# advimman/lama

Measured on NVIDIA H100. Metric: images/sec FFCResNetGenerator @512x512 bs32, higher is better.
Workload: dtype bf16x3(f32 accumulate)

## Files before the change

### include/ffc_b200.h

```cpp
#ifndef FFC_B200_H_
#define FFC_B200_H_

#include <stddef.h>
#include <stdint.h>

#ifdef __cplusplus
extern "C" {
#endif

#define FFCB_VERSION 117

enum {
  FFCB_OK = 0,
  FFCB_EINVAL = -1,
  FFCB_EARCH = -2,
  FFCB_ECUDA = -3,
  FFCB_ENOMEM = -4
};

enum { FFCB_F32 = 0, FFCB_BF16X2 = 1 };
enum { FFCB_ACT_NONE = 0, FFCB_ACT_RELU = 1, FFCB_ACT_SIGMOID = 2, FFCB_ACT_TANH = 3 };
enum { FFCB_BORDER_ZERO = 0, FFCB_BORDER_REFLECT = 1 };
enum {
  FFCB_MATH_FP32 = 0,
  FFCB_MATH_BF16X3 = 1
};

typedef void* ffcb_stream_t;

typedef struct {
  void* ptr;
  int64_t sb, sy, sx;
  int64_t lo_off;
  int32_t B, H, W, C;
  int32_t fmt;
  int32_t pad;
  int32_t reflect_border;
  int32_t window;
  int32_t cg;
  int32_t tile;
  int64_t sg;
} ffcb_tensor;

typedef struct {
  int32_t src, dy, dx, c0, nch;
} ffcb_kseg;

#define FFCB_MAX_KSEG 64

typedef struct {
  ffcb_tensor in[2];
  ffcb_tensor out;
  ffcb_tensor addend;
  const void* weight;
  const float* shift;
  int32_t n_out;
  int32_t stride;
  int32_t border;
  int32_t act;
  int32_t nseg;
  int32_t math;
  int32_t addend_post;
  int32_t _reserved;
  ffcb_kseg seg[FFCB_MAX_KSEG];
} ffcb_conv_desc;

int ffcb_version(void);
const char* ffcb_last_error(void);
int ffcb_check_device(int device);
void ffcb_shutdown(void);

int ffcb_conv(const ffcb_conv_desc* desc, ffcb_stream_t stream);

enum { FFCB_PLAN_FLAT = 0, FFCB_PLAN_SPATIAL = 1, FFCB_PLAN_ROWS = 2, FFCB_PLAN_HALO = 3 };
typedef struct {
  int32_t kind;
  int32_t il, po, ring;
  int32_t bn, tw, th, stages;
  int64_t m_tiles;
  int32_t n_tiles;
  int32_t _reserved;
} ffcb_conv_plan_info;
int ffcb_conv_plan(const ffcb_conv_desc* desc, ffcb_conv_plan_info* info);

int ffcb_stem_conv7(const float* x_nchw, int B, int Cin, int H, int W, const float* w, const float* shift,
                    int N, const ffcb_tensor* out, ffcb_stream_t stream);

int ffcb_stem_pack(const float* x_nchw, int B, int Cin, int H, int W, const ffcb_tensor* packed, ffcb_stream_t stream);

int ffcb_head_conv7(const ffcb_tensor* in, const float* w, const float* bias, int N, int act, float* y_nchw,
                    ffcb_stream_t stream);

size_t ffcb_fft2_workspace_bytes(int B, int H, int W, int C);
int ffcb_rfft2(const ffcb_tensor* in, const ffcb_tensor* spec, void* ws, size_t ws_bytes, ffcb_stream_t stream);
int ffcb_irfft2(const ffcb_tensor* spec, const ffcb_tensor* residual , const ffcb_tensor* out,
                void* ws, size_t ws_bytes, ffcb_stream_t stream);

int ffcb_head_gather7(const ffcb_tensor* q, const float* bias, int N, int act, float* y_nchw, ffcb_stream_t stream);

int ffcb_stem_pack_u8(const uint8_t* image_hwc, const uint8_t* mask_hw, int B, int H0, int W0,
                      const ffcb_tensor* packed, ffcb_stream_t stream);
int ffcb_head_gather7_blend_u8(const ffcb_tensor* q, const float* bias, int act, const uint8_t* image_hwc,
                               const uint8_t* mask_hw, int H0, int W0, uint8_t* out_hwc, ffcb_stream_t stream);

int ffcb_nchw_to_nhwc(const float* x_nchw, int B, int C, int H, int W, const ffcb_tensor* out, ffcb_stream_t stream);
int ffcb_nhwc_to_nchw(const ffcb_tensor* in, float* y_nchw, ffcb_stream_t stream);
int ffcb_fill_reflect_border(const ffcb_tensor* t, ffcb_stream_t stream);
// ... 34 lines not shown
```

### lama_b200/_lib.py

```python
import ctypes as C
import os

HERE = os.path.dirname(os.path.abspath(__file__))
LIB_PATH = os.path.join(HERE, "libffc_b200.so")

OK, EINVAL, EARCH, ECUDA, ENOMEM = 0, -1, -2, -3, -4
F32, BF16X2 = 0, 1
ACT_NONE, ACT_RELU, ACT_SIGMOID, ACT_TANH = 0, 1, 2, 3
BORDER_ZERO, BORDER_REFLECT = 0, 1
MATH_FP32, MATH_BF16X3 = 0, 1
MAX_KSEG = 64
PLAN_FLAT, PLAN_SPATIAL, PLAN_ROWS, PLAN_HALO = 0, 1, 2, 3
VERSION = 117


class Tensor(C.Structure):
    _fields_ = [("ptr", C.c_void_p), ("sb", C.c_int64), ("sy", C.c_int64), ("sx", C.c_int64),
                ("lo_off", C.c_int64), ("B", C.c_int32), ("H", C.c_int32), ("W", C.c_int32), ("C", C.c_int32),
                ("fmt", C.c_int32), ("pad", C.c_int32), ("reflect_border", C.c_int32), ("window", C.c_int32),
                ("cg", C.c_int32), ("tile", C.c_int32), ("sg", C.c_int64)]


class KSeg(C.Structure):
    _fields_ = [("src", C.c_int32), ("dy", C.c_int32), ("dx", C.c_int32), ("c0", C.c_int32), ("nch", C.c_int32)]


class ConvDesc(C.Structure):
    _fields_ = [("inp", Tensor * 2), ("out", Tensor), ("addend", Tensor), ("weight", C.c_void_p),
                ("shift", C.c_void_p), ("n_out", C.c_int32), ("stride", C.c_int32), ("border", C.c_int32),
                ("act", C.c_int32), ("nseg", C.c_int32), ("math", C.c_int32), ("addend_post", C.c_int32),
                ("_reserved", C.c_int32), ("seg", KSeg * MAX_KSEG)]


class ConvPlanInfo(C.Structure):
    _fields_ = [("kind", C.c_int32), ("il", C.c_int32), ("po", C.c_int32), ("ring", C.c_int32), ("bn", C.c_int32),
                ("tw", C.c_int32), ("th", C.c_int32), ("stages", C.c_int32), ("m_tiles", C.c_int64),
                ("n_tiles", C.c_int32), ("_reserved", C.c_int32)]


_PT = C.POINTER(Tensor)
SIGNATURES = {
    "ffcb_version": (C.c_int, []),
    "ffcb_last_error": (C.c_char_p, []),
    "ffcb_check_device": (C.c_int, [C.c_int]),
    "ffcb_shutdown": (None, []),
    "ffcb_conv": (C.c_int, [C.POINTER(ConvDesc), C.c_void_p]),
# ... 69 lines not shown
```

### lama_b200/csrc/conv_tc.cu

```cuda
#include <cuda.h>
#include <stdlib.h>

#include <type_traits>

#include "common.cuh"

namespace ffcb {
namespace {

constexpr int BM = 128;
constexpr int BK = 64;
constexpr int WG_K = 16;
constexpr int kThreads = 384;
constexpr int kConsumers = 256;
constexpr int kTileABytes = BM * BK * 2;
constexpr int kMaxStages = 8;
constexpr int kBarBytes = 1024;
constexpr int kSmemLimit = 227 * 1024;

struct TcParams {
  View out, addend;
  const float* shift;
  int N, act, addend_post;
  int BN, num_n_tiles;
// ... 140 lines not shown
__device__ __forceinline__ void wgmma_n128(float* d, uint64_t da, uint64_t db, uint32_t scale_d) {
  asm volatile(
      "{\n\t.reg .pred p;\n\tsetp.ne.b32 p, %66, 0;\n\t"
      "wgmma.mma_async.sync.aligned.m64n128k16.f32.bf16.bf16 {"
      "%0, %1, %2, %3, %4, %5, %6, %7, %8, %9, %10, %11, %12, %13, %14, %15, "
      "%16, %17, %18, %19, %20, %21, %22, %23, %24, %25, %26, %27, %28, %29, %30, %31, "
      "%32, %33, %34, %35, %36, %37, %38, %39, %40, %41, %42, %43, %44, %45, %46, %47, "
      "%48, %49, %50, %51, %52, %53, %54, %55, %56, %57, %58, %59, %60, %61, %62, %63"
      "}, %64, %65, p, 1, 1, 0, 0;\n\t}\n"
      : "+f"(d[0]), "+f"(d[1]), "+f"(d[2]), "+f"(d[3]), "+f"(d[4]), "+f"(d[5]), "+f"(d[6]), "+f"(d[7]),
        "+f"(d[8]), "+f"(d[9]), "+f"(d[10]), "+f"(d[11]), "+f"(d[12]), "+f"(d[13]), "+f"(d[14]), "+f"(d[15]),
        "+f"(d[16]), "+f"(d[17]), "+f"(d[18]), "+f"(d[19]), "+f"(d[20]), "+f"(d[21]), "+f"(d[22]), "+f"(d[23]),
        "+f"(d[24]), "+f"(d[25]), "+f"(d[26]), "+f"(d[27]), "+f"(d[28]), "+f"(d[29]), "+f"(d[30]), "+f"(d[31]),
        "+f"(d[32]), "+f"(d[33]), "+f"(d[34]), "+f"(d[35]), "+f"(d[36]), "+f"(d[37]), "+f"(d[38]), "+f"(d[39]),
        "+f"(d[40]), "+f"(d[41]), "+f"(d[42]), "+f"(d[43]), "+f"(d[44]), "+f"(d[45]), "+f"(d[46]), "+f"(d[47]),
        "+f"(d[48]), "+f"(d[49]), "+f"(d[50]), "+f"(d[51]), "+f"(d[52]), "+f"(d[53]), "+f"(d[54]), "+f"(d[55]),
        "+f"(d[56]), "+f"(d[57]), "+f"(d[58]), "+f"(d[59]), "+f"(d[60]), "+f"(d[61]), "+f"(d[62]), "+f"(d[63])
      : "l"(da), "l"(db), "r"(scale_d));
}
template <int BN>
__device__ __forceinline__ void wgmma_bn(float* d, uint64_t da, uint64_t db, uint32_t scale_d) {
  static_assert(BN == 32 || BN == 64 || BN == 96 || BN == 128, "N tile");
  if constexpr (BN == 32) wgmma_n32(d, da, db, scale_d);
  else if constexpr (BN == 64) wgmma_n64(d, da, db, scale_d);
  else if constexpr (BN == 96) wgmma_n96(d, da, db, scale_d);
  else wgmma_n128(d, da, db, scale_d);
}

struct TileCoord {
  int b, y0, x0;
  long long m0;
};

__device__ __forceinline__ TileCoord tile_coord(const TcParams& p, long long m_tile) {
  TileCoord t;
  if (p.flat) {
    t.m0 = m_tile * BM;
    t.b = 0; t.y0 = 0; t.x0 = 0;
  } else {
    const int per_img = p.tiles_x * p.tiles_y;
    t.b = (int)(m_tile / per_img);
    const int r = (int)(m_tile - (long long)t.b * per_img);
    t.y0 = (r / p.tiles_x) * p.TH;
    t.x0 = (r % p.tiles_x) * p.TW;
    t.m0 = 0;
  }
  return t;
}

template <bool IL, bool PO, bool RR, bool HALO, int BN>
__global__ void __launch_bounds__(kThreads, 1)
conv_tc_kernel(const __grid_constant__ TcParams p, const __grid_constant__ CUtensorMap map_in0,
               const __grid_constant__ CUtensorMap map_in1, const __grid_constant__ CUtensorMap map_w) {
  extern __shared__ __align__(1024) uint8_t smem_raw[];
  uint8_t* smem = reinterpret_cast<uint8_t*>((reinterpret_cast<uintptr_t>(smem_raw) + 1023) & ~(uintptr_t)1023);
  const int w_bytes = p.BN * BK * 2;
  const int stage_bytes = RR ? 2 * p.rr_a_bytes : HALO ? 2 * w_bytes : 2 * kTileABytes + 2 * w_bytes;
  uint8_t* w_res = smem;
  uint8_t* a_buf = smem;
  if constexpr (RR) smem += p.rr_w_bytes;
  if constexpr (HALO) smem += (size_t)4 * p.halo_a_bytes;
  uint64_t* bars = reinterpret_cast<uint64_t*>(smem + (size_t)p.stages * stage_bytes);
  uint64_t* full = bars;
  uint64_t* empty = bars + kMaxStages;
  uint64_t* w_bar = bars + 2 * kMaxStages;
  uint64_t* a_full = bars + 2 * kMaxStages + 1;
  uint64_t* a_empty = a_full + 2;

  const int warp = threadIdx.x >> 5, lane = threadIdx.x & 31;

  if (warp == 0 && lane == 0) {
    prefetch_tmap(&map_in0);
    prefetch_tmap(&map_in1);
    prefetch_tmap(&map_w);
  }
  if (warp == 1 && lane == 0) {
    for (int s = 0; s < p.stages; ++s) { mbar_init(&full[s], 1); mbar_init(&empty[s], kConsumers); }
    if constexpr (RR) mbar_init(w_bar, 1);
    if constexpr (HALO)
      for (int s = 0; s < 2; ++s) { mbar_init(&a_full[s], 1); mbar_init(&a_empty[s], kConsumers); }
// ... 96 lines not shown
              uint8_t* st = smem + (size_t)stage * stage_bytes;
              mbar_expect_tx(&full[stage], (uint32_t)stage_bytes);
              const int cc = g.c0 + j * BK;
              if (IL && il) {
                const long long blk = p.flat ? (tc.m0 >> 7)
                                             : (long long)tc.b * p.a_tiles_per_image[g.src] + ((tc.y0 * p.out.W) >> 7);
                const unsigned short* src = p.a_ptr[g.src] + blk * p.a_sg[g.src] + (long long)(cc >> 3) * 1024;
                bulk_load(st, src, kTileABytes, &full[stage]);
                bulk_load(st + kTileABytes, src + p.a_lo[g.src], kTileABytes, &full[stage]);
              } else if (p.flat) {
                tma_load_3d(st, map, &full[stage], cc, (int)tc.m0, 0);
                tma_load_3d(st + kTileABytes, map, &full[stage], cc, (int)tc.m0, 1);
              } else {
                tma_load_5d(st, map, &full[stage], cc, cx, cy, tc.b, 0);
                tma_load_5d(st + kTileABytes, map, &full[stage], cc, cx, cy, tc.b, 1);
              }
              tma_load_3d(st + 2 * kTileABytes, &map_w, &full[stage], kb * BK, n_tile * p.BN, 0);
              tma_load_3d(st + 2 * kTileABytes + w_bytes, &map_w, &full[stage], kb * BK, n_tile * p.BN, 1);
            }
            __syncwarp();
            if (++stage == p.stages) { stage = 0; phase ^= 1; }
          }
        }
      }
    }
  } else if (warp >= 4) {
    const int g = (warp >> 2) - 1;
    const int w = warp & 3, q = lane & 3;
    const int row = g * 64 + w * 16 + (lane >> 2) + 8 * (q & 1);
    const int cb = 4 * (q >> 1);
    const bool odd = (q & 1) != 0;
    const uint32_t a_row_sw = (uint32_t)(g * 64 * BK * 2) >> 4;
    const uint32_t a_row_il = (uint32_t)(g * 64 * 16) >> 4;
    const int HW = p.out.H * p.out.W;
    const bool has_add = p.addend.ptr != nullptr;
    float acc[BN / 2];
#pragma unroll
    for (int i = 0; i < BN / 2; ++i) acc[i] = 0.f;
    int stage = 0, ast = 0;
    uint32_t phase = 0, aph = 0;
    const int a_row0 = (g + 1) * p.TW;
    if constexpr (RR) mbar_wait(w_bar, 0);
    for (long long t = blockIdx.x; t < num_tiles; t += gridDim.x) {
      const int n_tile = (int)(t % p.num_n_tiles);
      const TileCoord tc = tile_coord(p, t / p.num_n_tiles);
      fence_acc<BN>(acc);
      if constexpr (HALO) {
        int prev = -1, a_prev = -1, nt = 0;
        for (int s = 0; s < p.nseg;) {
          const int ntap = p.seg_taps[s];
          const int nblk = (p.seg[s].nch + BK - 1) / BK;
          for (int j = 0; j < nblk; ++j) {
            for (int u = 0; u < (ntap == 9 ? 3 : 1); ++u) {
              const int dxu = ntap == 9 ? u - 1 : p.seg[s].dx;
              mbar_wait(&a_full[ast], aph);
              const uint32_t ab = smem_u32(a_buf + (size_t)ast * 2 * p.halo_a_bytes);
              for (int tap = 0; tap < ntap; ++tap) {
                const int dy = p.seg[s + tap].dy;
                if (p.seg[s + tap].dx != dxu) continue;
                const uint32_t a_off = (uint32_t)((a_row0 + dy * p.TW) * (BK * 2)) >> 4;
                const uint32_t a_hi = desc_addr(ab) + a_off;
                const uint32_t a_lo = desc_addr(ab + (uint32_t)p.halo_a_bytes) + a_off;
                mbar_wait(&full[stage], phase);
                wgmma_fence();
                const uint32_t st = smem_u32(smem + (size_t)stage * stage_bytes);
                const uint32_t w_hi = desc_addr(st), w_lo = desc_addr(st + (uint32_t)w_bytes);
#pragma unroll
                for (int k = 0; k < BK / WG_K; ++k) {
// ... 51 lines not shown
        for (int kb = 0; kb < total_kblocks; ++kb) {
          const bool il = IL && p.a_il[p.seg[sgi].src] != 0;
          const uint32_t a_lodesc = il ? kLoIl : kLoSw, a_hidesc = il ? kHiIl : kHiSw;
          const uint32_t a_row = il ? a_row_il : a_row_sw;
          const uint32_t a_step = il ? (uint32_t)(4096 >> 4) : (uint32_t)((WG_K * 2) >> 4);
          if (IL && ++j == (p.seg[sgi].nch + BK - 1) / BK) { ++sgi; j = 0; }
          mbar_wait(&full[stage], phase);
          wgmma_fence();
          const uint32_t st = smem_u32(smem + (size_t)stage * stage_bytes);
          const uint32_t a_hi = desc_addr(st) + a_row;
          const uint32_t a_lo = desc_addr(st + kTileABytes) + a_row;
          const uint32_t w_hi = desc_addr(st + 2 * kTileABytes);
          const uint32_t w_lo = desc_addr(st + 2 * kTileABytes + w_bytes);
#pragma unroll
          for (int k = 0; k < BK / WG_K; ++k) {
            const uint32_t wadv = (uint32_t)((k * WG_K * 2) >> 4);
            const uint32_t aadv = (uint32_t)k * a_step;
            wgmma_bn<BN>(acc, desc64((a_hi + aadv) | a_lodesc, a_hidesc), desc64((w_hi + wadv) | kLoSw, kHiSw),
                         (kb | k) != 0);
            wgmma_bn<BN>(acc, desc64((a_lo + aadv) | a_lodesc, a_hidesc), desc64((w_hi + wadv) | kLoSw, kHiSw), 1);
            wgmma_bn<BN>(acc, desc64((a_hi + aadv) | a_lodesc, a_hidesc), desc64((w_lo + wadv) | kLoSw, kHiSw), 1);
          }
          wgmma_commit();
          wgmma_wait<1>();
          if (prev >= 0) mbar_arrive(&empty[prev]);
          prev = stage;
          if (++stage == p.stages) { stage = 0; phase ^= 1; }
        }
        wgmma_wait<0>();
        fence_acc<BN>(acc);
        mbar_arrive(&empty[prev]);
      }

      int b, y, x;
      bool valid;
      if (p.flat) {
        const unsigned m = (unsigned)tc.m0 + (unsigned)row;
        valid = m < (unsigned)(p.out.B * HW);
        const unsigned mm = valid ? m : 0u;
        b = (int)(mm / (unsigned)HW);
        const unsigned r = mm - (unsigned)b * (unsigned)HW;
        y = (int)(r / (unsigned)p.out.W);
        x = (int)(r - (unsigned)y * (unsigned)p.out.W);
      } else {
        b = tc.b;
        y = tc.y0 + row / p.TW;
        x = tc.x0 + row % p.TW;
        valid = y < p.out.H && x < p.out.W;
      }
      const long long o_out = valid ? pix_off(p.out, b, y, x) : 0;
      const long long o_add = (has_add && valid) ? pix_off(p.addend, b, y, x) : 0;
      int mir_dy = 0, mir_dx = 0;
      if (!PO && p.ring && valid) {
        int my, mx;
        if (ring_mirrors(p.out, y, x, my, mx)) {
          if (my != -2) mir_dy = (my - y) * (int)p.out.sy;
          if (mx != -2) mir_dx = (mx - x) * (int)p.out.sx;
        }
      }
      const uint64_t pol = l2_policy(PO && p.hints ? 2 : 0);
      constexpr int EB = (BN / 8) % 8 == 0 ? 8 : 4;
      static_assert((BN / 8) % EB == 0, "whole batches of column groups");
#pragma unroll
      for (int j0 = 0; j0 < BN / 8; j0 += EB) {
        float4 shv[EB], adv[EB];
#pragma unroll
        for (int i = 0; i < EB; ++i) {
          const int n = n_tile * p.BN + 8 * (j0 + i) + cb;
          const bool ok = valid && n < p.N;
          shv[i] = (ok && p.shift != nullptr) ? __ldg(reinterpret_cast<const float4*>(p.shift + n))
                                               : make_float4(0.f, 0.f, 0.f, 0.f);
          adv[i] = (ok && has_add) ? load4(p.addend, o_add + n) : make_float4(0.f, 0.f, 0.f, 0.f);
        }
#pragma unroll
        for (int i = 0; i < EB; ++i) {
          const int j = j0 + i;
          const float s0 = odd ? acc[4 * j] : acc[4 * j + 2], s1 = odd ? acc[4 * j + 1] : acc[4 * j + 3];
          const float r0 = __shfl_xor_sync(0xffffffffu, s0, 1), r1 = __shfl_xor_sync(0xffffffffu, s1, 1);
          float4 v = odd ? make_float4(r0, r1, acc[4 * j + 2], acc[4 * j + 3])
                         : make_float4(acc[4 * j], acc[4 * j + 1], r0, r1);
          const int n = n_tile * p.BN + 8 * j + cb;
          if (!valid || n >= p.N) continue;
          const float4 sh = shv[i], ad = adv[i];
          v.x += sh.x; v.y += sh.y; v.z += sh.z; v.w += sh.w;
          if (!p.addend_post) { v.x += ad.x; v.y += ad.y; v.z += ad.z; v.w += ad.w; }
          if (p.act == FFCB_ACT_RELU) {
            v.x = fmaxf(v.x, 0.f); v.y = fmaxf(v.y, 0.f); v.z = fmaxf(v.z, 0.f); v.w = fmaxf(v.w, 0.f);
          } else if (p.act != FFCB_ACT_NONE) {
            v.x = slow_act(v.x, p.act); v.y = slow_act(v.y, p.act); v.z = slow_act(v.z, p.act); v.w = slow_act(v.w, p.act);
          }
          if (p.addend_post) { v.x += ad.x; v.y += ad.y; v.z += ad.z; v.w += ad.w; }
          if constexpr (PO) {
            st_hint_f4(reinterpret_cast<float*>(p.out.ptr) + o_out + chan_off(p.out, n), v, pol);
          } else {
            store4(p.out, o_out + n, v);
            if (mir_dy) store4(p.out, o_out + mir_dy + n, v);
            if (mir_dx) store4(p.out, o_out + mir_dx + n, v);
            if (mir_dy && mir_dx) store4(p.out, o_out + mir_dy + mir_dx + n, v);
          }
        }
      }
    }
  }
}

typedef CUresult (*EncodeTiledFn)(CUtensorMap*, CUtensorMapDataType, cuuint32_t, void*, const cuuint64_t*,
                                  const cuuint64_t*, const cuuint32_t*, const cuuint32_t*, CUtensorMapInterleave,
                                  CUtensorMapSwizzle, CUtensorMapL2promotion, CUtensorMapFloatOOBfill);

EncodeTiledFn get_encode() {
  static EncodeTiledFn fn = nullptr;
  if (fn == nullptr) {
    void* p = nullptr;
    cudaDriverEntryPointQueryResult q;
    if (cudaGetDriverEntryPoint("cuTensorMapEncodeTiled", &p, cudaEnableDefault, &q) == cudaSuccess &&
        q == cudaDriverEntryPointSuccess)
      fn = reinterpret_cast<EncodeTiledFn>(p);
  }
  return fn;
}

int encode_typed(CUtensorMap* map, void* base, CUtensorMapDataType dt, CUtensorMapSwizzle sw, int rank,
                 const cuuint64_t* dims, const cuuint64_t* strides_bytes, const cuuint32_t* box, const cuuint32_t* estr,
                 const char* what) {
  EncodeTiledFn fn = get_encode();
  if (fn == nullptr) {
    set_error("conv(tc): cuTensorMapEncodeTiled entry point unavailable");
    return FFCB_ECUDA;
  }
  CUresult r = fn(map, dt, (cuuint32_t)rank, base, dims, strides_bytes, box, estr, CU_TENSOR_MAP_INTERLEAVE_NONE, sw,
                  CU_TENSOR_MAP_L2_PROMOTION_L2_256B, CU_TENSOR_MAP_FLOAT_OOB_FILL_NONE);
  if (r != CUDA_SUCCESS) {
    set_error("conv(tc): cuTensorMapEncodeTiled(%s) failed with CUresult %d (rank %d, dims %llu %llu %llu, box %u %u %u)",
              what, (int)r, rank, (unsigned long long)dims[0], (unsigned long long)dims[1],
// ... 127 lines not shown
    rr = rr && (rr_dy_max - rr_dy_min) <= 8;
    const char* etw = getenv("FFCB_TC_ROWS_TW");
    rr_tw = (etw && atoi(etw) == 16) ? 16 : 8;
    if (rr) {
      const int w_res = d->nseg * 2 * p.BN * BK * 2;
      const int halo_stage = 2 * (BM / rr_tw + rr_dy_max - rr_dy_min) * rr_tw * BK * 2;
      rr = (kSmemLimit - 1024 - kBarBytes - w_res) / halo_stage >= 2;
    }
  }
  bool halo = !flat && !rr && d->stride == 1 && W > 32 && d->out.cg == 0;
  int ngroups = 0;
  for (int i = 0; i < d->nseg && halo;) {
    const ffcb_kseg& g = d->seg[i];
    const ffcb_tensor& t = d->in[g.src];
    halo = t.cg == 0 && d->border == FFCB_BORDER_REFLECT && taps[g.src] && t.pad >= 1 && t.window == 0;
    unsigned mask = 0;
    int n = 0;
    for (; n < 9 && i + n < d->nseg; ++n) {
      const ffcb_kseg& q = d->seg[i + n];
      if (q.src != g.src || q.c0 != g.c0 || q.nch != g.nch || q.dy < -1 || q.dy > 1 || q.dx < -1 || q.dx > 1) break;
      mask |= 1u << ((q.dy + 1) * 3 + q.dx + 1);
    }
    if (n == 9 && mask == 0x1FFu) {
      p.seg_taps[i] = 9;
      for (int k = 1; k < 9; ++k) p.seg_taps[i + k] = 0;
      i += 9;
      ++ngroups;
    } else {
      halo = halo && g.dy >= -1 && g.dy <= 1 && g.dx >= -1 && g.dx <= 1;
      p.seg_taps[i++] = 1;
    }
  }
  halo = halo && ngroups > 0;
  p.halo_a_bytes = 0;
  if (flat) {
    p.TW = BM; p.TH = 1; p.tiles_x = p.tiles_y = 1;
    p.num_m_tiles = ((long long)d->out.B * H * W + BM - 1) / BM;
  } else if (rr) {
    p.TW = rr_tw;
    p.TH = BM / p.TW;
    p.tiles_x = (W + p.TW - 1) / p.TW;
    p.tiles_y = (H + p.TH - 1) / p.TH;
    p.num_m_tiles = (long long)d->out.B * p.tiles_x * p.tiles_y;
    p.rr_dy0 = rr_dy_min;
    p.rr_a_bytes = (p.TH + rr_dy_max - rr_dy_min) * p.TW * BK * 2;
    p.rr_w_bytes = d->nseg * 2 * p.BN * BK * 2;
  } else if (halo) {
    p.TW = 64; p.TH = 2;
    p.tiles_x = (W + p.TW - 1) / p.TW;
    p.tiles_y = (H + p.TH - 1) / p.TH;
    p.num_m_tiles = (long long)d->out.B * p.tiles_x * p.tiles_y;
    p.halo_a_bytes = p.TW * (p.TH + 2) * BK * 2;
  } else {
    int tw = 1;
    while (tw < W && tw < BM) tw <<= 1;
    p.TW = tw; p.TH = BM / tw;
    p.tiles_x = (W + p.TW - 1) / p.TW;
    p.tiles_y = (H + p.TH - 1) / p.TH;
    p.num_m_tiles = (long long)d->out.B * p.tiles_x * p.tiles_y;
    FFCB_REQUIRE(p.TW * d->stride <= 256 && p.TH * d->stride <= 256, "conv(tc): tile exceeds the TMA box limit");
  }

  for (int s = 0; s < 2; ++s)
    if (p.a_il[s] && !flat)
      FFCB_REQUIRE(p.TW == W && p.TW * p.TH == BM && H % p.TH == 0 && (H * W) % BM == 0,
                   "conv(tc): tile-blocked in[%d] in a spatial contraction needs M tiles of whole rows (W a power of two "
                   "<= 128 dividing 128, H*W a multiple of 128); got %dx%d", s, H, W);
  for (int s = 0; s < 2; ++s)
    p.coord_off[s] = (used[s] && !p.a_il[s] && !flat && taps[s] && d->border == FFCB_BORDER_REFLECT) ? d->in[s].pad : 0;
  FFCB_REQUIRE(((uintptr_t)d->weight % 16) == 0, "conv(tc): weight pointer not 16-byte aligned");
  if (d->out.cg == 0) {
    const ffcb_tensor& t = d->out;
    const int64_t esz = t.fmt == FFCB_BF16X2 ? 2 : 4;
    FFCB_REQUIRE(((uintptr_t)t.ptr % 16) == 0 && (t.sx * esz) % 16 == 0 && (t.sy * esz) % 16 == 0 &&
                     (t.sb * esz) % 16 == 0 && (esz == 4 || (t.lo_off * esz) % 16 == 0),
                 "conv(tc): out strides / pointer not 16-byte aligned (C must be a multiple of %d)", esz == 2 ? 8 : 4);
  }

  pl.stage_bytes = rr ? 2 * p.rr_a_bytes : halo ? 2 * p.BN * BK * 2 : 2 * kTileABytes + 2 * p.BN * BK * 2;
  pl.bar_bytes = kBarBytes + (rr ? p.rr_w_bytes : 0) + (halo ? 4 * p.halo_a_bytes : 0);
  int stages = (kSmemLimit - 1024 - pl.bar_bytes) / pl.stage_bytes;
  if (stages > kMaxStages) stages = kMaxStages;
  FFCB_REQUIRE(stages >= 2, "conv(tc): BN=%d leaves fewer than 2 pipeline stages", p.BN);
  p.stages = stages;
  pl.smem = (size_t)stages * pl.stage_bytes + pl.bar_bytes + 1024;

  pl.kind = flat ? FFCB_PLAN_FLAT : rr ? FFCB_PLAN_ROWS : halo ? FFCB_PLAN_HALO : FFCB_PLAN_SPATIAL;
  pl.il = !rr && !halo && (p.a_il[0] || p.a_il[1]);
  pl.po = p.out_planar != 0;
  pl.rr_span = rr ? rr_dy_max - rr_dy_min : 0;
  pl.kpad = kpad;
  return FFCB_OK;
}

}

int conv_tc_plan(const ffcb_conv_desc* d, ffcb_conv_plan_info* info) {
  TcPlan pl;
  const int rc = plan_tc(d, pl);
  if (rc) return rc;
  info->kind = pl.kind;
  info->il = pl.il;
  info->po = pl.po;
  info->ring = pl.p.ring;
  info->bn = pl.p.BN;
  info->tw = pl.p.TW;
  info->th = pl.p.TH;
  info->stages = pl.p.stages;
  info->m_tiles = pl.p.num_m_tiles;
  info->n_tiles = pl.p.num_n_tiles;
  info->_reserved = 0;
  return FFCB_OK;
}

int conv_tc(const ffcb_conv_desc* d, cudaStream_t stream) {
  TcPlan pl;
  int rc = plan_tc(d, pl);
  if (rc) return rc;
  TcParams& p = pl.p;
  const bool rr = pl.kind == FFCB_PLAN_ROWS, halo = pl.kind == FFCB_PLAN_HALO, flat = pl.kind == FFCB_PLAN_FLAT;

  alignas(64) CUtensorMap maps[3];
  for (int s = 0; s < 2; ++s) {
    if (!pl.used[s] || p.a_il[s]) continue;
    const ffcb_tensor& t = d->in[s];
    const cuuint64_t esz = 2;
    if (flat) {
      cuuint64_t dims[3] = {(cuuint64_t)t.C, (cuuint64_t)t.B * t.H * t.W, 2};
      cuuint64_t str[2] = {(cuuint64_t)t.sx * esz, (cuuint64_t)t.lo_off * esz};
      cuuint32_t box[3] = {BK, BM, 1}, es[3] = {1, 1, 1};
      if ((rc = encode(&maps[s], t.ptr, 3, dims, str, box, es, "flat activations"))) return rc;
    } else {
      const int off = p.coord_off[s];
      char* base = (char*)t.ptr - (int64_t)off * ((int64_t)t.sy + t.sx) * (int64_t)esz;
      cuuint64_t dims[5] = {(cuuint64_t)t.C, (cuuint64_t)(t.W + 2 * off), (cuuint64_t)(t.H + 2 * off),
                            (cuuint64_t)t.B, 2};
      cuuint64_t str[4] = {(cuuint64_t)t.sx * esz, (cuuint64_t)t.sy * esz, (cuuint64_t)t.sb * esz,
                           (cuuint64_t)t.lo_off * esz};
      cuuint32_t box[5] = {BK, (cuuint32_t)(p.TW * d->stride), (cuuint32_t)(p.TH * d->stride), 1, 1};
      if (rr) box[2] = (cuuint32_t)(p.TH + pl.rr_span);
      if (halo) box[2] = (cuuint32_t)(p.TH + 2);
      cuuint32_t es[5] = {1, (cuuint32_t)d->stride, (cuuint32_t)d->stride, 1, 1};
      if ((rc = encode(&maps[s], base, 5, dims, str, box, es, "spatial activations"))) return rc;
    }
  }
  {
    cuuint64_t dims[3] = {(cuuint64_t)pl.kpad, (cuuint64_t)d->n_out, 2};
    cuuint64_t str[2] = {(cuuint64_t)pl.kpad * 2, (cuuint64_t)pl.kpad * d->n_out * 2};
    cuuint32_t box[3] = {BK, (cuuint32_t)p.BN, 1}, es[3] = {1, 1, 1};
    if ((rc = encode(&maps[2], const_cast<void*>(d->weight), 3, dims, str, box, es, "weights"))) return rc;
  }
  for (int s = 0; s < 2; ++s)
    if (!pl.used[s] || p.a_il[s]) maps[s] = maps[2];

  int dev = 0, sms = 132;
  FFCB_CUDA(cudaGetDevice(&dev));
  FFCB_CUDA(cudaDeviceGetAttribute(&sms, cudaDevAttrMultiProcessorCount, dev));
  const long long tiles = p.num_m_tiles * p.num_n_tiles;
  const int grid = (int)(tiles < sms ? tiles : sms);
  const size_t smem = pl.smem;
  auto launch = [&](auto kernel) -> int {
    FFCB_CUDA(cudaFuncSetAttribute(kernel, cudaFuncAttributeMaxDynamicSharedMemorySize, kSmemLimit));
    kernel<<<grid, kThreads, smem, stream>>>(p, maps[0], maps[1], maps[2]);
    return FFCB_OK;
  };
  auto launch_bn = [&](auto bn) -> int {
    constexpr int N = decltype(bn)::value;
    if (rr) return launch(conv_tc_kernel<false, false, true, false, N>);
    if (halo) return launch(conv_tc_kernel<false, false, false, true, N>);
    if (pl.il)
      return pl.po ? launch(conv_tc_kernel<true, true, false, false, N>)
                   : launch(conv_tc_kernel<true, false, false, false, N>);
    return pl.po ? launch(conv_tc_kernel<false, true, false, false, N>)
                 : launch(conv_tc_kernel<false, false, false, false, N>);
  };
  switch (p.BN) {
    case 32: rc = launch_bn(std::integral_constant<int, 32>()); break;
    case 64: rc = launch_bn(std::integral_constant<int, 64>()); break;
    case 96: rc = launch_bn(std::integral_constant<int, 96>()); break;
    default: rc = launch_bn(std::integral_constant<int, 128>()); break;
  }
  if (rc) return rc;
  FFCB_LAUNCH_CHECK("conv_tc_kernel");
  return FFCB_OK;
}

}
```

Baseline: 335.4.

## Add weight-stationary streaming conv kernel with M=64 tiles and per-warpgroup pipelines

Adds a new conv plan in which each CTA keeps its whole N-tile of weights (hi/lo bf16 split) resident in shared memory for the entire K, loaded once. Activations stream through per-consumer-warpgroup rings of 64-row, half-BK stages using 64B swizzle. Two producer/consumer warpgroup pairs work on interleaved M tiles. The goal is to stop reloading weights for every M tile and to raise pipeline depth. The risks are a smaller wgmma M per warpgroup, more barrier traffic, and a plan selected by default through a heuristic that the 2x-SM tile threshold gates. The epilogue is factored into a shared helper.

```diff
diff --git a/include/ffc_b200.h b/include/ffc_b200.h
--- a/include/ffc_b200.h
+++ b/include/ffc_b200.h
@@ -8,7 +8,7 @@
 extern "C" {
 #endif
 
-#define FFCB_VERSION 117
+#define FFCB_VERSION 118
 
 enum {
   FFCB_OK = 0,
@@ -72,7 +72,7 @@
 
 int ffcb_conv(const ffcb_conv_desc* desc, ffcb_stream_t stream);
 
-enum { FFCB_PLAN_FLAT = 0, FFCB_PLAN_SPATIAL = 1, FFCB_PLAN_ROWS = 2, FFCB_PLAN_HALO = 3 };
+enum { FFCB_PLAN_FLAT = 0, FFCB_PLAN_SPATIAL = 1, FFCB_PLAN_ROWS = 2, FFCB_PLAN_HALO = 3, FFCB_PLAN_STREAM = 4 };
 typedef struct {
   int32_t kind;
   int32_t il, po, ring;
diff --git a/lama_b200/_lib.py b/lama_b200/_lib.py
--- a/lama_b200/_lib.py
+++ b/lama_b200/_lib.py
@@ -10,8 +10,8 @@
 BORDER_ZERO, BORDER_REFLECT = 0, 1
 MATH_FP32, MATH_BF16X3 = 0, 1
 MAX_KSEG = 64
-PLAN_FLAT, PLAN_SPATIAL, PLAN_ROWS, PLAN_HALO = 0, 1, 2, 3
-VERSION = 117
+PLAN_FLAT, PLAN_SPATIAL, PLAN_ROWS, PLAN_HALO, PLAN_STREAM = 0, 1, 2, 3, 4
+VERSION = 118
 
 
 class Tensor(C.Structure):
diff --git a/lama_b200/csrc/conv_tc.cu b/lama_b200/csrc/conv_tc.cu
--- a/lama_b200/csrc/conv_tc.cu
+++ b/lama_b200/csrc/conv_tc.cu
@@ -196,10 +196,11 @@
   long long m0;
 };
 
+template <int TM = BM>
 __device__ __forceinline__ TileCoord tile_coord(const TcParams& p, long long m_tile) {
   TileCoord t;
   if (p.flat) {
-    t.m0 = m_tile * BM;
+    t.m0 = m_tile * TM;
     t.b = 0; t.y0 = 0; t.x0 = 0;
   } else {
     const int per_img = p.tiles_x * p.tiles_y;
@@ -210,6 +211,81 @@
     t.m0 = 0;
   }
   return t;
+}
+
+template <bool PO, int BN>
+__device__ __forceinline__ void tile_epilogue(const TcParams& p, const float* acc, const TileCoord& tc, int n_tile,
+                                              int row, int cb, bool odd) {
+  const int HW = p.out.H * p.out.W;
+  const bool has_add = p.addend.ptr != nullptr;
+  int b, y, x;
+  bool valid;
+  if (p.flat) {
+    const unsigned m = (unsigned)tc.m0 + (unsigned)row;
+    valid = m < (unsigned)(p.out.B * HW);
+    const unsigned mm = valid ? m : 0u;
+    b = (int)(mm / (unsigned)HW);
+    const unsigned r = mm - (unsigned)b * (unsigned)HW;
+    y = (int)(r / (unsigned)p.out.W);
+    x = (int)(r - (unsigned)y * (unsigned)p.out.W);
+  } else {
+    b = tc.b;
+    y = tc.y0 + row / p.TW;
+    x = tc.x0 + row % p.TW;
+    valid = y < p.out.H && x < p.out.W;
+  }
+  const long long o_out = valid ? pix_off(p.out, b, y, x) : 0;
+  const long long o_add = (has_add && valid) ? pix_off(p.addend, b, y, x) : 0;
+  int mir_dy = 0, mir_dx = 0;
+  if (!PO && p.ring && valid) {
+    int my, mx;
+    if (ring_mirrors(p.out, y, x, my, mx)) {
+      if (my != -2) mir_dy = (my - y) * (int)p.out.sy;
+      if (mx != -2) mir_dx = (mx - x) * (int)p.out.sx;
+    }
+  }
+  const uint64_t pol = l2_policy(PO && p.hints ? 2 : 0);
+  constexpr int EB = (BN / 8) % 8 == 0 ? 8 : 4;
+  static_assert((BN / 8) % EB == 0, "whole batches of column groups");
+#pragma unroll
+  for (int j0 = 0; j0 < BN / 8; j0 += EB) {
+    float4 shv[EB], adv[EB];
+#pragma unroll
+    for (int i = 0; i < EB; ++i) {
+      const int n = n_tile * p.BN + 8 * (j0 + i) + cb;
+      const bool ok = valid && n < p.N;
+      shv[i] = (ok && p.shift != nullptr) ? __ldg(reinterpret_cast<const float4*>(p.shift + n))
+                                           : make_float4(0.f, 0.f, 0.f, 0.f);
+      adv[i] = (ok && has_add) ? load4(p.addend, o_add + n) : make_float4(0.f, 0.f, 0.f, 0.f);
+    }
+#pragma unroll
+    for (int i = 0; i < EB; ++i) {
+      const int j = j0 + i;
+      const float s0 = odd ? acc[4 * j] : acc[4 * j + 2], s1 = odd ? acc[4 * j + 1] : acc[4 * j + 3];
+      const float r0 = __shfl_xor_sync(0xffffffffu, s0, 1), r1 = __shfl_xor_sync(0xffffffffu, s1, 1);
+      float4 v = odd ? make_float4(r0, r1, acc[4 * j + 2], acc[4 * j + 3])
+                     : make_float4(acc[4 * j], acc[4 * j + 1], r0, r1);
+      const int n = n_tile * p.BN + 8 * j + cb;
+      if (!valid || n >= p.N) continue;
+      const float4 sh = shv[i], ad = adv[i];
+      v.x += sh.x; v.y += sh.y; v.z += sh.z; v.w += sh.w;
+      if (!p.addend_post) { v.x += ad.x; v.y += ad.y; v.z += ad.z; v.w += ad.w; }
+      if (p.act == FFCB_ACT_RELU) {
+        v.x = fmaxf(v.x, 0.f); v.y = fmaxf(v.y, 0.f); v.z = fmaxf(v.z, 0.f); v.w = fmaxf(v.w, 0.f);
+      } else if (p.act != FFCB_ACT_NONE) {
+        v.x = slow_act(v.x, p.act); v.y = slow_act(v.y, p.act); v.z = slow_act(v.z, p.act); v.w = slow_act(v.w, p.act);
+      }
+      if (p.addend_post) { v.x += ad.x; v.y += ad.y; v.z += ad.z; v.w += ad.w; }
+      if constexpr (PO) {
+        st_hint_f4(reinterpret_cast<float*>(p.out.ptr) + o_out + chan_off(p.out, n), v, pol);
+      } else {
+        store4(p.out, o_out + n, v);
+        if (mir_dy) store4(p.out, o_out + mir_dy + n, v);
+        if (mir_dx) store4(p.out, o_out + mir_dx + n, v);
+        if (mir_dy && mir_dx) store4(p.out, o_out + mir_dy + mir_dx + n, v);
+      }
+    }
+  }
 }
 
 template <bool IL, bool PO, bool RR, bool HALO, int BN>
@@ -372,8 +448,6 @@
     const bool odd = (q & 1) != 0;
     const uint32_t a_row_sw = (uint32_t)(g * 64 * BK * 2) >> 4;
     const uint32_t a_row_il = (uint32_t)(g * 64 * 16) >> 4;
-    const int HW = p.out.H * p.out.W;
-    const bool has_add = p.addend.ptr != nullptr;
     float acc[BN / 2];
 #pragma unroll
     for (int i = 0; i < BN / 2; ++i) acc[i] = 0.f;
@@ -491,74 +565,153 @@
         mbar_arrive(&empty[prev]);
       }
 
-      int b, y, x;
-      bool valid;
-      if (p.flat) {
-        const unsigned m = (unsigned)tc.m0 + (unsigned)row;
-        valid = m < (unsigned)(p.out.B * HW);
-        const unsigned mm = valid ? m : 0u;
-        b = (int)(mm / (unsigned)HW);
-        const unsigned r = mm - (unsigned)b * (unsigned)HW;
-        y = (int)(r / (unsigned)p.out.W);
-        x = (int)(r - (unsigned)y * (unsigned)p.out.W);
-      } else {
-        b = tc.b;
-        y = tc.y0 + row / p.TW;
-        x = tc.x0 + row % p.TW;
-        valid = y < p.out.H && x < p.out.W;
-      }
-      const long long o_out = valid ? pix_off(p.out, b, y, x) : 0;
-      const long long o_add = (has_add && valid) ? pix_off(p.addend, b, y, x) : 0;
-      int mir_dy = 0, mir_dx = 0;
-      if (!PO && p.ring && valid) {
-        int my, mx;
-        if (ring_mirrors(p.out, y, x, my, mx)) {
-          if (my != -2) mir_dy = (my - y) * (int)p.out.sy;
-          if (mx != -2) mir_dx = (mx - x) * (int)p.out.sx;
+      tile_epilogue<PO, BN>(p, acc, tc, n_tile, row, cb, odd);
+    }
+  }
+}
+
+constexpr int kStreamM = 64;
+constexpr int kStreamK = BK / 2;
+constexpr int kStreamABytes = kStreamM * kStreamK * 2;
+constexpr int kStreamMinRing = 4, kStreamMaxRing = 8;
+constexpr uint32_t kLoIl64 = (uint32_t)(1024 >> 4) << 16;
+constexpr uint32_t kHiSw64 = (uint32_t)(512 >> 4) | (2u << 30);
+
+template <bool IL, int BN>
+__global__ void __launch_bounds__(kThreads, 1)
+conv_tc_stream_kernel(const __grid_constant__ TcParams p, const __grid_constant__ CUtensorMap map_in0,
+                      const __grid_constant__ CUtensorMap map_in1, const __grid_constant__ CUtensorMap map_w) {
+  extern __shared__ __align__(1024) uint8_t smem_raw[];
+  uint8_t* smem = reinterpret_cast<uint8_t*>((reinterpret_cast<uintptr_t>(smem_raw) + 1023) & ~(uintptr_t)1023);
+  constexpr int w_bytes = BN * BK * 2;
+  int total_kblocks = 0;
+  for (int s = 0; s < p.nseg; ++s) total_kblocks += (p.seg[s].nch + BK - 1) / BK;
+  const int R = p.stages;
+  uint8_t* w_res = smem;
+  uint8_t* a_st = smem + (size_t)total_kblocks * 2 * w_bytes;
+  uint64_t* bars = reinterpret_cast<uint64_t*>(a_st + (size_t)2 * R * 2 * kStreamABytes);
+  uint64_t* full = bars;
+  uint64_t* empty = bars + 2 * kStreamMaxRing;
+  uint64_t* w_bar = bars + 4 * kStreamMaxRing;
+
+  const int warp = threadIdx.x >> 5, lane = threadIdx.x & 31;
+  const int n_tile = (int)(blockIdx.x % p.num_n_tiles);
+  const int slot = (int)(blockIdx.x / p.num_n_tiles);
+  const int workers = 2 * (int)(gridDim.x / p.num_n_tiles);
+
+  if (warp == 0 && lane == 0) {
+    prefetch_tmap(&map_in0);
+    prefetch_tmap(&map_in1);
+    prefetch_tmap(&map_w);
+  }
+  if (warp == 2 && lane == 0) {
+    for (int s = 0; s < 2 * R; ++s) { mbar_init(&full[s], 1); mbar_init(&empty[s], kConsumers / 2); }
+    mbar_init(w_bar, 1);
+    asm volatile("fence.mbarrier_init.release.cluster;" ::: "memory");
+  }
+  __syncthreads();
+
+  if (warp < 2) {
+    const int g = warp;
+    if (g == 0) {
+      if (elect_one()) {
+        mbar_expect_tx(w_bar, (uint32_t)(total_kblocks * 2 * w_bytes));
+        for (int kb = 0; kb < total_kblocks; ++kb) {
+          tma_load_3d(w_res + (size_t)kb * 2 * w_bytes, &map_w, w_bar, kb * BK, n_tile * BN, 0);
+          tma_load_3d(w_res + (size_t)kb * 2 * w_bytes + w_bytes, &map_w, w_bar, kb * BK, n_tile * BN, 1);
         }
       }
-      const uint64_t pol = l2_policy(PO && p.hints ? 2 : 0);
-      constexpr int EB = (BN / 8) % 8 == 0 ? 8 : 4;
-      static_assert((BN / 8) % EB == 0, "whole batches of column groups");
+      __syncwarp();
+    }
+    const int HW = p.out.H * p.out.W;
+    int stage = 0;
+    uint32_t phase = 0;
+    for (long long m = 2 * slot + g; m < p.num_m_tiles; m += workers) {
+      const TileCoord tc = tile_coord<kStreamM>(p, m);
+      for (int s = 0; s < p.nseg; ++s) {
+        const ffcb_kseg sg = p.seg[s];
+        const CUtensorMap* map = sg.src ? &map_in1 : &map_in0;
+        const int nblk = (sg.nch + BK - 1) / BK;
+        for (int j = 0; j < 2 * nblk; ++j) {
+          mbar_wait(&empty[g * R + stage], phase ^ 1);
+          if (elect_one()) {
+            uint8_t* st = a_st + (size_t)(g * R + stage) * 2 * kStreamABytes;
+            uint64_t* bar = &full[g * R + stage];
+            mbar_expect_tx(bar, 2u * kStreamABytes);
+            const int cc = sg.c0 + j * kStreamK;
+            if (IL && p.a_il[sg.src]) {
+              const long long px = p.flat ? tc.m0 : (long long)tc.b * HW + (long long)tc.y0 * p.out.W;
+              const unsigned short* src = p.a_ptr[sg.src] + (px >> 7) * p.a_sg[sg.src] + (long long)(cc >> 3) * 1024 +
+                                          (px & (BM - 1)) * 8;
 #pragma unroll
-      for (int j0 = 0; j0 < BN / 8; j0 += EB) {
-        float4 shv[EB], adv[EB];
-#pragma unroll
-        for (int i = 0; i < EB; ++i) {
-          const int n = n_tile * p.BN + 8 * (j0 + i) + cb;
-          const bool ok = valid && n < p.N;
-          shv[i] = (ok && p.shift != nullptr) ? __ldg(reinterpret_cast<const float4*>(p.shift + n))
-                                               : make_float4(0.f, 0.f, 0.f, 0.f);
-          adv[i] = (ok && has_add) ? load4(p.addend, o_add + n) : make_float4(0.f, 0.f, 0.f, 0.f);
-        }
-#pragma unroll
-        for (int i = 0; i < EB; ++i) {
-          const int j = j0 + i;
-          const float s0 = odd ? acc[4 * j] : acc[4 * j + 2], s1 = odd ? acc[4 * j + 1] : acc[4 * j + 3];
-          const float r0 = __shfl_xor_sync(0xffffffffu, s0, 1), r1 = __shfl_xor_sync(0xffffffffu, s1, 1);
-          float4 v = odd ? make_float4(r0, r1, acc[4 * j + 2], acc[4 * j + 3])
-                         : make_float4(acc[4 * j], acc[4 * j + 1], r0, r1);
-          const int n = n_tile * p.BN + 8 * j + cb;
-          if (!valid || n >= p.N) continue;
-          const float4 sh = shv[i], ad = adv[i];
-          v.x += sh.x; v.y += sh.y; v.z += sh.z; v.w += sh.w;
-          if (!p.addend_post) { v.x += ad.x; v.y += ad.y; v.z += ad.z; v.w += ad.w; }
-          if (p.act == FFCB_ACT_RELU) {
-            v.x = fmaxf(v.x, 0.f); v.y = fmaxf(v.y, 0.f); v.z = fmaxf(v.z, 0.f); v.w = fmaxf(v.w, 0.f);
-          } else if (p.act != FFCB_ACT_NONE) {
-            v.x = slow_act(v.x, p.act); v.y = slow_act(v.y, p.act); v.z = slow_act(v.z, p.act); v.w = slow_act(v.w, p.act);
+              for (int gi = 0; gi < kStreamK / 8; ++gi) {
+                bulk_load(st + gi * 1024, src + gi * 1024, 1024, bar);
+                bulk_load(st + kStreamABytes + gi * 1024, src + p.a_lo[sg.src] + gi * 1024, 1024, bar);
+              }
+            } else if (p.flat) {
+              tma_load_3d(st, map, bar, cc, (int)tc.m0, 0);
+              tma_load_3d(st + kStreamABytes, map, bar, cc, (int)tc.m0, 1);
+            } else {
+              tma_load_5d(st, map, bar, cc, tc.x0, tc.y0, tc.b, 0);
+              tma_load_5d(st + kStreamABytes, map, bar, cc, tc.x0, tc.y0, tc.b, 1);
+            }
           }
-          if (p.addend_post) { v.x += ad.x; v.y += ad.y; v.z += ad.z; v.w += ad.w; }
-          if constexpr (PO) {
-            st_hint_f4(reinterpret_cast<float*>(p.out.ptr) + o_out + chan_off(p.out, n), v, pol);
-          } else {
-            store4(p.out, o_out + n, v);
-            if (mir_dy) store4(p.out, o_out + mir_dy + n, v);
-            if (mir_dx) store4(p.out, o_out + mir_dx + n, v);
-            if (mir_dy && mir_dx) store4(p.out, o_out + mir_dy + mir_dx + n, v);
-          }
+          __syncwarp();
+          if (++stage == R) { stage = 0; phase ^= 1; }
         }
       }
+    }
+  } else if (warp >= 4) {
+    const int g = (warp >> 2) - 1;
+    const int w = warp & 3, q = lane & 3;
+    const int row = w * 16 + (lane >> 2) + 8 * (q & 1);
+    const int cb = 4 * (q >> 1);
+    const bool odd = (q & 1) != 0;
+    float acc[BN / 2];
+#pragma unroll
+    for (int i = 0; i < BN / 2; ++i) acc[i] = 0.f;
+    int stage = 0;
+    uint32_t phase = 0;
+    const uint32_t wr = smem_u32(w_res);
+    mbar_wait(w_bar, 0);
+    for (long long m = 2 * slot + g; m < p.num_m_tiles; m += workers) {
+      const TileCoord tc = tile_coord<kStreamM>(p, m);
+      fence_acc<BN>(acc);
+      int prev = -1, sgi = 0, j = 0;
+      for (int kb = 0; kb < total_kblocks; ++kb) {
+        const bool il = IL && p.a_il[p.seg[sgi].src] != 0;
+        const uint32_t a_lodesc = il ? kLoIl64 : kLoSw, a_hidesc = il ? kHiIl : kHiSw64;
+        const uint32_t a_step = il ? (uint32_t)(2048 >> 4) : (uint32_t)((WG_K * 2) >> 4);
+        if (IL && ++j == (p.seg[sgi].nch + BK - 1) / BK) { ++sgi; j = 0; }
+        const uint32_t w_hi = desc_addr(wr + (uint32_t)(kb * 2 * w_bytes));
+        const uint32_t w_lo = desc_addr(wr + (uint32_t)(kb * 2 * w_bytes + w_bytes));
+#pragma unroll
+        for (int h = 0; h < 2; ++h) {
+          mbar_wait(&full[g * R + stage], phase);
+          wgmma_fence();
+          const uint32_t st = smem_u32(a_st + (size_t)(g * R + stage) * 2 * kStreamABytes);
+          const uint32_t a_hi = desc_addr(st), a_lo = desc_addr(st + kStreamABytes);
+#pragma unroll
+          for (int kk = 0; kk < kStreamK / WG_K; ++kk) {
+            const int k = h * (kStreamK / WG_K) + kk;
+            const uint32_t wadv = (uint32_t)((k * WG_K * 2) >> 4);
+            const uint32_t aadv = (uint32_t)kk * a_step;
+            wgmma_bn<BN>(acc, desc64((a_hi + aadv) | a_lodesc, a_hidesc), desc64((w_hi + wadv) | kLoSw, kHiSw),
+                         (kb | k) != 0);
+            wgmma_bn<BN>(acc, desc64((a_lo + aadv) | a_lodesc, a_hidesc), desc64((w_hi + wadv) | kLoSw, kHiSw), 1);
+            wgmma_bn<BN>(acc, desc64((a_hi + aadv) | a_lodesc, a_hidesc), desc64((w_lo + wadv) | kLoSw, kHiSw), 1);
+          }
+          wgmma_commit();
+          wgmma_wait<1>();
+          if (prev >= 0) mbar_arrive(&empty[g * R + prev]);
+          prev = stage;
+          if (++stage == R) { stage = 0; phase ^= 1; }
+        }
+      }
+      wgmma_wait<0>();
+      fence_acc<BN>(acc);
+      mbar_arrive(&empty[g * R + prev]);
+      tile_epilogue<true, BN>(p, acc, tc, n_tile, row, cb, odd);
     }
   }
 }
@@ -752,8 +905,43 @@
     }
   }
   halo = halo && ngroups > 0;
+  bool stream = false;
+  int stream_tw = 1, stream_ring = 0;
+  {
+    const char* e = getenv("FFCB_TC_STREAM");
+    stream = (e ? atoi(e) != 0 : true) && d->out.cg != 0 && d->stride == 1 && !taps[0] && !taps[1];
+    while (stream_tw < W && stream_tw < kStreamM) stream_tw <<= 1;
+    for (int s = 0; s < 2 && stream; ++s)
+      if (used[s] && d->in[s].cg != 0)
+        stream = d->in[s].sg % 8 == 0 &&
+                 (flat || (stream_tw == W && H % (kStreamM / stream_tw) == 0 && (H * W) % BM == 0));
+    auto ring_depth = [&](int bn) {
+      const int r = (kSmemLimit - 1024 - kBarBytes - (kpad / BK) * 2 * bn * BK * 2) / (2 * 2 * kStreamABytes);
+      return r < kStreamMaxRing ? r : kStreamMaxRing;
+    };
+    int bn = p.BN;
+    if (getenv("FFCB_TC_BN") == nullptr)
+      while (bn > 32 && ring_depth(bn) < kStreamMinRing) bn -= 32;
+    const int nt = (d->n_out + bn - 1) / bn;
+    const long long mt = flat ? ((long long)d->out.B * H * W + kStreamM - 1) / kStreamM
+                              : (long long)d->out.B * ((W + stream_tw - 1) / stream_tw) *
+                                    ((H + kStreamM / stream_tw - 1) / (kStreamM / stream_tw));
+    stream = stream && ring_depth(bn) >= kStreamMinRing && nt <= 66 && mt * nt >= 4 * 2 * 132;
+    if (stream) {
+      p.BN = bn;
+      p.num_n_tiles = nt;
+      stream_ring = ring_depth(bn);
+    }
+  }
   p.halo_a_bytes = 0;
-  if (flat) {
+  if (stream) {
+    p.TW = flat ? kStreamM : stream_tw;
+    p.TH = flat ? 1 : kStreamM / stream_tw;
+    p.tiles_x = flat ? 1 : (W + p.TW - 1) / p.TW;
+    p.tiles_y = flat ? 1 : (H + p.TH - 1) / p.TH;
+    p.num_m_tiles = flat ? ((long long)d->out.B * H * W + kStreamM - 1) / kStreamM
+                         : (long long)d->out.B * p.tiles_x * p.tiles_y;
+  } else if (flat) {
     p.TW = BM; p.TH = 1; p.tiles_x = p.tiles_y = 1;
     p.num_m_tiles = ((long long)d->out.B * H * W + BM - 1) / BM;
   } else if (rr) {
@@ -782,7 +970,7 @@
   }
 
   for (int s = 0; s < 2; ++s)
-    if (p.a_il[s] && !flat)
+    if (p.a_il[s] && !flat && !stream)
       FFCB_REQUIRE(p.TW == W && p.TW * p.TH == BM && H % p.TH == 0 && (H * W) % BM == 0,
                    "conv(tc): tile-blocked in[%d] in a spatial contraction needs M tiles of whole rows (W a power of two "
                    "<= 128 dividing 128, H*W a multiple of 128); got %dx%d", s, H, W);
@@ -797,15 +985,19 @@
                  "conv(tc): out strides / pointer not 16-byte aligned (C must be a multiple of %d)", esz == 2 ? 8 : 4);
   }
 
-  pl.stage_bytes = rr ? 2 * p.rr_a_bytes : halo ? 2 * p.BN * BK * 2 : 2 * kTileABytes + 2 * p.BN * BK * 2;
-  pl.bar_bytes = kBarBytes + (rr ? p.rr_w_bytes : 0) + (halo ? 4 * p.halo_a_bytes : 0);
+  pl.stage_bytes = rr ? 2 * p.rr_a_bytes : halo ? 2 * p.BN * BK * 2 : stream ? 2 * kStreamABytes
+                                                                         : 2 * kTileABytes + 2 * p.BN * BK * 2;
+  pl.bar_bytes = kBarBytes + (rr ? p.rr_w_bytes : 0) + (halo ? 4 * p.halo_a_bytes : 0) +
+                 (stream ? (kpad / BK) * 2 * p.BN * BK * 2 : 0);
   int stages = (kSmemLimit - 1024 - pl.bar_bytes) / pl.stage_bytes;
   if (stages > kMaxStages) stages = kMaxStages;
   FFCB_REQUIRE(stages >= 2, "conv(tc): BN=%d leaves fewer than 2 pipeline stages", p.BN);
+  if (stream) stages = stream_ring;
   p.stages = stages;
-  pl.smem = (size_t)stages * pl.stage_bytes + pl.bar_bytes + 1024;
-
-  pl.kind = flat ? FFCB_PLAN_FLAT : rr ? FFCB_PLAN_ROWS : halo ? FFCB_PLAN_HALO : FFCB_PLAN_SPATIAL;
+  pl.smem = (size_t)(stream ? 2 * stages : stages) * pl.stage_bytes + pl.bar_bytes + 1024;
+
+  pl.kind = stream ? FFCB_PLAN_STREAM : flat ? FFCB_PLAN_FLAT : rr ? FFCB_PLAN_ROWS : halo ? FFCB_PLAN_HALO
+                                                                                          : FFCB_PLAN_SPATIAL;
   pl.il = !rr && !halo && (p.a_il[0] || p.a_il[1]);
   pl.po = p.out_planar != 0;
   pl.rr_span = rr ? rr_dy_max - rr_dy_min : 0;
@@ -838,7 +1030,8 @@
   int rc = plan_tc(d, pl);
   if (rc) return rc;
   TcParams& p = pl.p;
-  const bool rr = pl.kind == FFCB_PLAN_ROWS, halo = pl.kind == FFCB_PLAN_HALO, flat = pl.kind == FFCB_PLAN_FLAT;
+  const bool rr = pl.kind == FFCB_PLAN_ROWS, halo = pl.kind == FFCB_PLAN_HALO, streams = pl.kind == FFCB_PLAN_STREAM;
+  const bool flat = p.flat != 0;
 
   alignas(64) CUtensorMap maps[3];
   for (int s = 0; s < 2; ++s) {
@@ -848,8 +1041,12 @@
     if (flat) {
       cuuint64_t dims[3] = {(cuuint64_t)t.C, (cuuint64_t)t.B * t.H * t.W, 2};
       cuuint64_t str[2] = {(cuuint64_t)t.sx * esz, (cuuint64_t)t.lo_off * esz};
-      cuuint32_t box[3] = {BK, BM, 1}, es[3] = {1, 1, 1};
-      if ((rc = encode(&maps[s], t.ptr, 3, dims, str, box, es, "flat activations"))) return rc;
+      cuuint32_t box[3] = {(cuuint32_t)(streams ? kStreamK : BK), (cuuint32_t)(streams ? kStreamM : BM), 1};
+      cuuint32_t es[3] = {1, 1, 1};
+      if ((rc = encode_typed(&maps[s], t.ptr, CU_TENSOR_MAP_DATA_TYPE_BFLOAT16,
+                             streams ? CU_TENSOR_MAP_SWIZZLE_64B : CU_TENSOR_MAP_SWIZZLE_128B, 3, dims, str, box, es,
+                             "flat activations")))
+        return rc;
     } else {
       const int off = p.coord_off[s];
       char* base = (char*)t.ptr - (int64_t)off * ((int64_t)t.sy + t.sx) * (int64_t)esz;
@@ -857,11 +1054,15 @@
                             (cuuint64_t)t.B, 2};
       cuuint64_t str[4] = {(cuuint64_t)t.sx * esz, (cuuint64_t)t.sy * esz, (cuuint64_t)t.sb * esz,
                            (cuuint64_t)t.lo_off * esz};
-      cuuint32_t box[5] = {BK, (cuuint32_t)(p.TW * d->stride), (cuuint32_t)(p.TH * d->stride), 1, 1};
+      cuuint32_t box[5] = {(cuuint32_t)(streams ? kStreamK : BK), (cuuint32_t)(p.TW * d->stride),
+                           (cuuint32_t)(p.TH * d->stride), 1, 1};
       if (rr) box[2] = (cuuint32_t)(p.TH + pl.rr_span);
       if (halo) box[2] = (cuuint32_t)(p.TH + 2);
       cuuint32_t es[5] = {1, (cuuint32_t)d->stride, (cuuint32_t)d->stride, 1, 1};
-      if ((rc = encode(&maps[s], base, 5, dims, str, box, es, "spatial activations"))) return rc;
+      if ((rc = encode_typed(&maps[s], base, CU_TENSOR_MAP_DATA_TYPE_BFLOAT16,
+                             streams ? CU_TENSOR_MAP_SWIZZLE_64B : CU_TENSOR_MAP_SWIZZLE_128B, 5, dims, str, box, es,
+                             "spatial activations")))
+        return rc;
     }
   }
   {
@@ -877,7 +1078,13 @@
   FFCB_CUDA(cudaGetDevice(&dev));
   FFCB_CUDA(cudaDeviceGetAttribute(&sms, cudaDevAttrMultiProcessorCount, dev));
   const long long tiles = p.num_m_tiles * p.num_n_tiles;
-  const int grid = (int)(tiles < sms ? tiles : sms);
+  int grid = (int)(tiles < sms ? tiles : sms);
+  if (streams) {
+    FFCB_REQUIRE(sms >= p.num_n_tiles, "conv(tc): %d N tiles on %d SMs", p.num_n_tiles, sms);
+    long long slots = sms / p.num_n_tiles;
+    if (slots > (p.num_m_tiles + 1) / 2) slots = (p.num_m_tiles + 1) / 2;
+    grid = (int)slots * p.num_n_tiles;
+  }
   const size_t smem = pl.smem;
   auto launch = [&](auto kernel) -> int {
     FFCB_CUDA(cudaFuncSetAttribute(kernel, cudaFuncAttributeMaxDynamicSharedMemorySize, kSmemLimit));
@@ -886,6 +1093,8 @@
   };
   auto launch_bn = [&](auto bn) -> int {
     constexpr int N = decltype(bn)::value;
+    if (streams)
+      return pl.il ? launch(conv_tc_stream_kernel<true, N>) : launch(conv_tc_stream_kernel<false, N>);
     if (rr) return launch(conv_tc_kernel<false, false, true, false, N>);
     if (halo) return launch(conv_tc_kernel<false, false, false, true, N>);
     if (pl.il)
```

Result: no change. 336.1, median of 6 (+0.2%).
